# joybio/multiPrime

Measured on NVIDIA B200. Metric: candidate_x_sequence_evals_per_sec, higher is better.
Workload: dtype u32

## Files before the change

include/mpb200.h:

```cpp
#ifndef MPB200_H
#define MPB200_H

#include <stdint.h>

#ifdef __cplusplus
extern "C" {
#endif

#define MPB_ABI_VERSION 3
#define MPB_MAX_K 27
#define MPB_MAX_EXPANSIONS 65536

#define MPB_OK 0
#define MPB_EINVAL (-1)
#define MPB_ECUDA (-2)
#define MPB_ENOMEM (-3)
#define MPB_EOVERFLOW (-4)
#define MPB_EEXPAND (-5)

typedef struct mpb_ctx mpb_ctx;
typedef struct mpb_msa mpb_msa;
typedef struct mpb_hist mpb_hist;

int mpb_abi_version(void);
const char* mpb_last_error(void);
int mpb_device_count(void);

int mpb_ctx_create(int device, mpb_ctx** out);
void mpb_ctx_destroy(mpb_ctx* ctx);
int mpb_ctx_set_stream(mpb_ctx* ctx, void* cuda_stream);
int mpb_ctx_sync(mpb_ctx* ctx);
int64_t mpb_ctx_launches(mpb_ctx* ctx);
int mpb_dev_alloc(mpb_ctx* ctx, int64_t bytes, void** out);
void mpb_dev_free(mpb_ctx* ctx, void* p);
int mpb_ctx_memcpy(mpb_ctx* ctx, void* dst, const void* src, int64_t bytes);

int mpb_ctx_profile(mpb_ctx* ctx, int enable);
int mpb_ctx_profile_read(mpb_ctx* ctx, const char* kernel, double* ms, int64_t* launches, double* units);

int mpb_msa_upload(mpb_ctx* ctx, const uint8_t* packed4_hd, int64_t n_seq, int64_t n_col, int64_t row_bytes,
                   const int32_t* lens, mpb_msa** out);
void mpb_msa_free(mpb_msa* msa);
int64_t mpb_msa_nseq(const mpb_msa* msa);

int mpb_msa_set_row0(mpb_msa* msa, int64_t row0);

int mpb_seq_attr(mpb_msa* msa, int32_t* lead_gaps_hd, int32_t* rstrip_len_hd);

int mpb_window_prefilter(mpb_msa* msa, int k, int v, const int32_t* win_pos, int32_t nw, double* s0_hd, double* s1_hd);

int mpb_seq_attr_hist(mpb_msa* msa, int64_t* lead_hist_hd, int64_t* rstrip_hist_hd);

int mpb_hist_build(mpb_msa* msa, int k, int v, const int32_t* win_pos, int32_t nw, int log2_cap, mpb_hist** out);
void mpb_hist_free(mpb_hist* h);

int mpb_hist_create_empty(mpb_msa* msa, int k, int v, const int32_t* win_pos, int32_t nw, int log2_cap, mpb_hist** out);
int mpb_hist_add_counts(mpb_hist* h, const int64_t* gap_n, const int64_t* n_iupac_gap);

int mpb_hist_counts(mpb_hist* h, int64_t* gap_n, int64_t* n_iupac_gap, int64_t* n_entries);

int mpb_hist_export(mpb_hist* h, const uint8_t* sel, const int64_t* win_off, uint64_t* keys_hd, uint32_t* cnt_hd,
                    uint64_t* first_hd);

int mpb_hist_export_at(mpb_hist* h, int32_t n_sel, const int32_t* sel_idx, const int64_t* start, const int64_t* room,
                       int64_t total, uint64_t* keys_hd, uint32_t* cnt_hd, uint64_t* first_hd);

int mpb_hist_merge(mpb_hist* h, const int64_t* win_off, const uint64_t* keys_hd, const uint32_t* cnt_hd,
                   const uint64_t* first_hd);

int mpb_hist_summary(mpb_hist* h, int64_t* gap_n, double* ent, int64_t* nuniq, uint64_t* mm_key, int64_t* mm_cnt,
                     uint64_t* mm_first, int64_t* n_iupac_gap, int64_t* freq, int64_t* nn);

int mpb_hist_merge_segments(mpb_hist* h, int32_t n_seg, const int64_t* seg_off, const uint64_t* keys_hd,
                            const uint32_t* cnt_hd, const uint64_t* first_hd);

int mpb_hist_stats(mpb_hist* h, int64_t* gap_n, double* ent, int64_t* nuniq, uint64_t* mm_key, int64_t* mm_cnt,
                   uint64_t* mm_first, int64_t* n_iupac_gap);

int mpb_hist_tensors(mpb_hist* h, const uint8_t* sel, int64_t* freq_hd, int64_t* nn_hd);

int mpb_hist_dump(mpb_hist* h, int32_t w, int64_t max_n, uint64_t* keys_hd, uint32_t* cnt_hd, uint64_t* first_hd,
                  int64_t* n_out);
// ... 92 lines not shown
```

multiprime_b200/_lib.py:

```python
from __future__ import annotations

import ctypes as C
import os

import numpy as np

_PKG = os.path.dirname(os.path.abspath(__file__))
LIB_PATH = os.path.join(_PKG, "libmpb200.so")

MAX_K = 27
KEY_EMPTY = 0xFFFFFFFFFFFFFFFF
KEY_IUPAC = 0xFFFFFFFFFFFFFFFE
KEY_BASE5 = 1 << 54

_lib = None

_P = C.c_void_p
SIGNATURES = {
    "mpb_abi_version": (C.c_int, []),
    "mpb_last_error": (C.c_char_p, []),
    "mpb_device_count": (C.c_int, []),
    "mpb_ctx_create": (C.c_int, [C.c_int, C.POINTER(_P)]),
    "mpb_ctx_destroy": (None, [_P]),
    "mpb_ctx_set_stream": (C.c_int, [_P, _P]),
    "mpb_ctx_sync": (C.c_int, [_P]),
    "mpb_ctx_launches": (C.c_int64, [_P]),
    "mpb_ctx_memcpy": (C.c_int, [_P, _P, _P, C.c_int64]),
    "mpb_dev_alloc": (C.c_int, [_P, C.c_int64, C.POINTER(_P)]),
    "mpb_dev_free": (None, [_P, _P]),
    "mpb_ctx_profile": (C.c_int, [_P, C.c_int]),
    "mpb_ctx_profile_read": (C.c_int, [_P, C.c_char_p, C.POINTER(C.c_double), C.POINTER(C.c_int64),
                                        C.POINTER(C.c_double)]),
    "mpb_msa_upload": (C.c_int, [_P, _P, C.c_int64, C.c_int64, C.c_int64, _P, C.POINTER(_P)]),
    "mpb_msa_free": (None, [_P]),
    "mpb_msa_nseq": (C.c_int64, [_P]),
    "mpb_msa_set_row0": (C.c_int, [_P, C.c_int64]),
    "mpb_hist_counts": (C.c_int, [_P, _P, _P, _P]),
    "mpb_hist_export": (C.c_int, [_P, _P, _P, _P, _P, _P]),
    "mpb_seq_attr": (C.c_int, [_P, _P, _P]),
    "mpb_seq_attr_hist": (C.c_int, [_P, _P, _P]),
    "mpb_window_prefilter": (C.c_int, [_P, C.c_int, C.c_int, _P, C.c_int32, _P, _P]),
    "mpb_hist_build": (C.c_int, [_P, C.c_int, C.c_int, _P, C.c_int32, C.c_int, C.POINTER(_P)]),
    "mpb_hist_free": (None, [_P]),
    "mpb_hist_merge": (C.c_int, [_P, _P, _P, _P, _P]),
    "mpb_hist_stats": (C.c_int, [_P, _P, _P, _P, _P, _P, _P, _P]),
    "mpb_hist_tensors": (C.c_int, [_P, _P, _P, _P]),
    "mpb_hist_dump": (C.c_int, [_P, C.c_int32, C.c_int64, _P, _P, _P, C.POINTER(C.c_int64)]),
    "mpb_hist_match": (C.c_int, [_P, _P, _P, C.c_int32, _P]),
    "mpb_hist_exceptions": (C.c_int, [_P, C.c_int64, _P, _P, C.POINTER(C.c_int64)]),
    "mpb_scan": (C.c_int, [_P, C.c_int, C.c_int, C.c_uint32, C.c_uint32, _P, _P, C.c_int64, _P, _P, _P]),
    "mpb_pattern_hits": (C.c_int, [_P, C.c_int32, _P, _P, C.c_int64, _P, _P, _P, C.POINTER(C.c_int64)]),
    "mpb_seqkeys": (C.c_int, [_P, C.c_int, _P, C.c_int32, _P]),
    "mpb_tm": (C.c_int, [_P, _P, C.c_int, C.c_int64, _P, _P, _P, _P]),
    "mpb_tm_sets": (C.c_int, [_P, _P, C.c_int, C.c_int32, _P, _P, _P]),
    "mpb_walk": (C.c_int, [C.c_int, C.c_int, C.c_int, C.c_int, C.c_int32, _P, _P, _P, _P, _P, _P,
                           _P, _P, _P, _P, _P, C.c_int64, _P, _P, _P]),
    "mpb_hist_export_at": (C.c_int, [_P, C.c_int32, _P, _P, _P, C.c_int64, _P, _P, _P]),
    "mpb_hist_merge_segments": (C.c_int, [_P, C.c_int32, _P, _P, _P, _P]),
    "mpb_hist_create_empty": (C.c_int, [_P, C.c_int, C.c_int, _P, C.c_int32, C.c_int, C.POINTER(_P)]),
    "mpb_hist_add_counts": (C.c_int, [_P, _P, _P]),
    "mpb_hist_summary": (C.c_int, [_P, _P, _P, _P, _P, _P, _P, _P, _P, _P]),
    "mpb_cscan": (C.c_int, [_P, C.c_uint32, C.c_uint32, _P, C.c_int64, _P, _P, _P]),
    "mpb_walk_dev_begin": (C.c_int, [_P, C.c_int, C.c_int, C.c_uint32, C.c_uint32, C.c_int32, _P, _P, _P, _P, _P,
                                      C.POINTER(_P)]),
    "mpb_walk_dev_advance": (C.c_int, [_P]),
    "mpb_walk_dev_scan": (C.c_int, [_P]),
    "mpb_walk_dev_round": (C.c_int, [_P]),
    "mpb_walk_dev_counts": (C.c_int, [_P, C.POINTER(_P), C.POINTER(C.c_int64)]),
    "mpb_walk_dev_live": (C.c_int64, [_P]),
    "mpb_walk_dev_max_rounds": (C.c_int, [_P]),
    "mpb_walk_dev_wait": (C.c_int, [_P, C.c_int, C.POINTER(C.c_int64)]),
    "mpb_walk_dev_run": (C.c_int, [_P, C.c_int, C.POINTER(C.c_int64)]),
    "mpb_walk_dev_finish": (C.c_int, [_P, _P, _P, _P, _P, _P, C.c_int64, _P, _P, _P]),
    "mpb_walk_dev_free": (None, [_P]),
# ... 261 lines not shown
class Msa:

    def __init__(self, ctx: Context, packed4, n_seq: int, n_col: int, row_bytes: int | None = None, lens=None):
        self.ctx = ctx
        self.n_seq, self.n_col = int(n_seq), int(n_col)
        row_bytes = row_bytes if row_bytes is not None else (n_col + 1) // 2
        if lens is not None:
            lens = np.ascontiguousarray(lens, dtype=np.int32)
        h = C.c_void_p()
        check(load().mpb_msa_upload(ctx.h, ptr(packed4), n_seq, n_col, row_bytes, ptr(lens), C.byref(h)))
        self.h = h

    def close(self):
        if self.h:
            load().mpb_msa_free(self.h)
            self.h = None

    def set_row0(self, row0: int):
        check(load().mpb_msa_set_row0(self.h, row0))

    def seq_attr(self):
        lead = np.empty(self.n_seq, np.int32)
        rstrip = np.empty(self.n_seq, np.int32)
        check(load().mpb_seq_attr(self.h, ptr(lead), ptr(rstrip)))
        return lead, rstrip

    def prefilter(self, k: int, v: int, win_pos):
        win_pos = np.ascontiguousarray(win_pos, dtype=np.int32)
        s0 = np.zeros(len(win_pos), np.float64)
        s1 = np.zeros(len(win_pos), np.float64)
        check(load().mpb_window_prefilter(self.h, k, v, ptr(win_pos), len(win_pos), ptr(s0), ptr(s1)))
        return s0, s1

    def seq_attr_hist(self):
        lead = np.zeros(self.n_col + 1, np.int64)
        rstrip = np.zeros(self.n_col + 1, np.int64)
        check(load().mpb_seq_attr_hist(self.h, ptr(lead), ptr(rstrip)))
        return lead, rstrip

    def hist(self, k: int, v: int, win_pos, log2_cap: int = 0, empty: bool = False) -> "Hist":
        return Hist(self, k, v, win_pos, log2_cap, empty)

    def scan(self, k: int, v: int, fmask: int, rmask: int, cand_pos, cand_allow, bits_slot=None, counts_out=None,
             bits_out=None):
        cand_pos = np.ascontiguousarray(cand_pos, dtype=np.int32)
        cand_allow = np.ascontiguousarray(cand_allow, dtype=np.uint32).reshape(-1, 4)
        nc = len(cand_pos)
        counts = counts_out if counts_out is not None else np.zeros((nc, 3), np.int64)
        bits = bits_out
        if bits_slot is not None:
            bits_slot = np.ascontiguousarray(bits_slot, dtype=np.int32)
            nslots = int(bits_slot.max()) + 1 if nc else 0
            words = (self.n_seq + 31) // 32
            if bits is None:
                bits = np.zeros((max(nslots, 0), 3, words), np.uint32)
        if nc:
            check(load().mpb_scan(self.h, k, v, fmask, rmask, ptr(cand_pos), ptr(cand_allow), nc, ptr(counts),
                                  ptr(bits_slot), ptr(bits)))
        return counts, bits

    def pattern_hits(self, allow, lens, max_hits: int = 1 << 20):
        allow = np.ascontiguousarray(allow, dtype=np.uint32).reshape(-1, 4)
        lens = np.ascontiguousarray(lens, dtype=np.int32)
        while True:
            hp, hr, hx = (np.empty(max_hits, np.int32) for _ in range(3))
            n = C.c_int64()
            check(load().mpb_pattern_hits(self.h, len(lens), ptr(allow), ptr(lens), max_hits, ptr(hp), ptr(hr), ptr(hx),
                                          C.byref(n)))
            if n.value <= max_hits:
                break
            max_hits = int(n.value) + 16
        n = n.value
        order = np.lexsort((hx[:n], hr[:n], hp[:n]))
        return hp[:n][order], hr[:n][order], hx[:n][order]

    def seqkeys(self, k: int, win_pos) -> np.ndarray:
        win_pos = np.ascontiguousarray(win_pos, dtype=np.int32)
        out = np.empty((len(win_pos), self.n_seq), np.uint64)
        check(load().mpb_seqkeys(self.h, k, ptr(win_pos), len(win_pos), ptr(out)))
        return out


class Hist:

    def __init__(self, msa: Msa, k: int, v: int, win_pos, log2_cap: int = 0, empty: bool = False):
        self.msa = msa
        self.k, self.v = k, v
        self.win_pos = np.ascontiguousarray(win_pos, dtype=np.int32)
        self.nw = len(self.win_pos)
        self.h = None
        cap = log2_cap
        if empty:
            h = C.c_void_p()
            check(load().mpb_hist_create_empty(msa.h, k, v, ptr(self.win_pos), self.nw, cap, C.byref(h)))
            self.h = h
            self.log2_cap = cap
            return
        while True:
            h = C.c_void_p()
            rc = load().mpb_hist_build(msa.h, k, v, ptr(self.win_pos), self.nw, cap, C.byref(h))
            if rc == -4:
                if cap == 0:
                    cap = max(6, int(np.ceil(np.log2(2 * msa.n_seq + 64))))
                cap += 1
                continue
            check(rc)
            self.h = h
            self.log2_cap = cap
            break

    def close(self):
        if self.h:
            load().mpb_hist_free(self.h)
            self.h = None

    def __enter__(self):
        return self

    def __exit__(self, *a):
        self.close()

    def summary(self):
        nw, k = self.nw, self.k
        out = dict(gap_n=np.empty(nw, np.int64), ent=np.empty((nw, 4), np.float64), nuniq=np.empty((nw, 3), np.int64),
                   mm_key=np.empty(nw, np.uint64), mm_cnt=np.empty(nw, np.int64), mm_first=np.empty(nw, np.uint64),
                   n_iupac_gap=np.empty(nw, np.int64), freq=np.empty((nw, 4, k), np.int64),
                   nn=np.empty((nw, k - 1, 4, 4), np.int64))
        check(load().mpb_hist_summary(self.h, ptr(out["gap_n"]), ptr(out["ent"]), ptr(out["nuniq"]), ptr(out["mm_key"]),
                                      ptr(out["mm_cnt"]), ptr(out["mm_first"]), ptr(out["n_iupac_gap"]),
                                      ptr(out["freq"]), ptr(out["nn"])))
        return out

    def add_counts(self, gap_n, n_iupac_gap):
        gap_n = np.ascontiguousarray(gap_n, dtype=np.int64)
        n_iupac_gap = np.ascontiguousarray(n_iupac_gap, dtype=np.int64)
        check(load().mpb_hist_add_counts(self.h, ptr(gap_n), ptr(n_iupac_gap)))

# ... 347 lines not shown
```

multiprime_b200/core.py:

```python
from __future__ import annotations

import json
import math
import os
import sys
import time
from statistics import mean

import numpy as np

from . import _lib
from .comm import NoComm
from .iupac import BASES, CODE_CHARS, CHAR_CODE, allow_masks, expand_array, expand_keys, expand_strings, primer_string, rc_sets

TSV_HEADER = ["Position", "Entropy of cover (bit)", "Entropy of total (bit)", "Optimal_primer",
              "primer_degenerate_number", "nonsense_primer_number", "Optimal_coverage", "Mis-F-coverage",
              "Mis-R-coverage", "Tm", "Information"]


def _byte_table() -> bytes:
    t = bytearray(256)
    for ch, code in CHAR_CODE.items():
        if ch in "ACGTRYMKSWHBVD":
            t[ord(ch)] = code
# ... 315 lines not shown
        if row is None:
            if self._codes is not None:
                row = self._codes[s, :self.lens[s]].tobytes()
            else:
                pk = self._packed4[s]
                cells = np.empty(pk.shape[0] * 2, np.uint8)
                cells[0::2] = pk & 15
                cells[1::2] = pk >> 4
                row = cells[:self.lens[s]].tobytes()
            if len(self._row_cache) < 200000:
                self._row_cache[s] = row
        gap = b"\x00"
        w = row[p:p + k]
        if w != gap * k:
            if w.startswith(gap):
                body = w.lstrip(gap)
                g = len(w) - len(body)
                left = row[0:p].replace(gap, b"")
                if len(left) >= g:
                    w = left[len(left) - g:] + body
            if w.endswith(gap):
                body = w.rstrip(gap)
                g = len(w) - len(body)
                right = row[p + k:].replace(gap, b"")
                if len(right) >= g:
                    w = body + right[0:g]
        if len(w) < k:
            g = k - len(w)
            left = row[0:p].replace(gap, b"")
            if len(left) >= g:
                w = left[len(left) - g:] + w
        return w

    def _table_log2cap(self, k: int, n: int) -> int:
        if k < 8 or n < (1 << 17) or self.entropy_threshold > 4.0:
            return 0
        return max(10, int(math.ceil(math.log2(n / 2))))

    def design(self, positions):
        positions = [int(p) for p in positions]
        self.bit_vectors = []
        if not positions:
            return []
        per_batch = min(65535, self.windows_per_batch or _default_batch(self.n_local))
        out = []
        for b0 in range(0, len(positions), per_batch):
            out.extend(self._design_batch(positions[b0:b0 + per_batch]))
        return out

    def _design_batch(self, positions):
        k, v, N = self.primer_length, self.variation, self.total_sequence_number
        comm = self.comm
        self.stats["windows"] += len(positions)
        ph = self.stats.setdefault("phase_ms", {})
        tick = [time.perf_counter()]

        def lap(name):
            now = time.perf_counter()
            ph[name] = ph.get(name, 0.0) + 1000 * (now - tick[0])
            tick[0] = now

        if k >= 8:
            if self.n_local > 0:
                s0, s1 = self.msa.prefilter(k, v, positions)
                bound = (s0 * math.log2(self.n_local) - s1) / N
            else:
                bound = np.zeros(len(positions))
            if comm.world > 1:
                bound = comm.allreduce_sum(bound)
            keep_pos = bound <= self.entropy_threshold + 0.006
        else:
            keep_pos = np.ones(len(positions), bool)
        self.stats["prefiltered"] = self.stats.get("prefiltered", 0) + int((~keep_pos).sum())
        positions = [p for p, kp in zip(positions, keep_pos.tolist()) if kp]
        lap("prefilter")
        if not positions:
            return []
        owner = (np.arange(len(positions)) % comm.world).astype(np.int32)
        with self.msa.hist(k, v, positions, self._table_log2cap(k, self.n_local)) as hist:
            lap("hist_build")
            own = None
            try:
                if comm.world > 1:
                    st, own, mine = self._exchange(hist, positions, owner)
                    lap("exchange")
                else:
                    st, mine = hist.stats(), None
                    lap("summary")
                out = self._gates_walk_finish(hist, own, mine, owner, st, positions, lap)
            finally:
                if own is not None:
                    own.close()
        lap("free")
        return out

    def _gates_walk_finish(self, hist, own, mine, owner, st, positions, lap):
        k, v, N = self.primer_length, self.variation, self.total_sequence_number
        comm = self.comm
        gap_n = st["gap_n"]
        ratio = gap_n / N
        gap_fail = np.round(ratio, 2) >= (1 - self.coverage)
        for wi in np.nonzero(np.abs((ratio * 100) % 1 - 0.5) < 1e-6)[0]:
            gap_fail[wi] = round(int(gap_n[wi]) / N, 2) >= (1 - self.coverage)
        alive = ~gap_fail & (st["nuniq"][:, 0] >= 1)
        accepted = []
        for wi, ent in self._entropies(hist, own, mine, owner, st, positions, alive):
            accepted.append((wi, positions[wi], ent[0], ent[1], N - int(gap_n[wi]), bool(st["nuniq"][wi, 2] > 0)))
        lap("gates")
        if not accepted:
            return []
        if "freq" in st:
            freq, nn = st["freq"], st["nn"]
# ... 465 lines not shown
```

multiprime_b200/csrc/mpb200.cu:

```cuda
#include <cuda_runtime.h>
#include <stdint.h>
#include <stdarg.h>
#include <stdio.h>
#include <string.h>

#include <string>
#include <algorithm>
#include <vector>

#include "mpb200.h"
#include "mpb_host.h"
#include "mpb_device.cuh"
#include "mpb_prefilter.h"

static thread_local std::string g_err;

int mpb_fail(int code, const char* fmt, ...) {
    char buf[512];
    va_list ap;
    va_start(ap, fmt);
    vsnprintf(buf, sizeof buf, fmt, ap);
    va_end(ap);
    g_err = buf;
    return code;
// ... 793 lines not shown
                        }
                        qn += __popc(mm);
                        __syncwarp();
                    }
                }
                if (late)
                    hist_row(pl, nsp, s, len, p, k, v, kmask, row0, wi, K, C, F, E, log2cap, gap_n, iupac_gap_n, exc, exc_n,
                             exc_max, n_entries, gap_bits, nwords, spec_win, spec_row, spec_n, spec_cap, late_special ? 1 : 0, err);
            }
        }
        if (lane < gr.y) {
            const int wi = gr.x + lane;
            if (my_count)
                mpb_table_add(keys + (uint64_t)wi * cap, cnt + (uint64_t)wi * cap, first + (uint64_t)wi * cap, log2cap, my_major,
                              my_count, my_first, err, &n_entries[wi], elist + (uint64_t)wi * cap);
            if (my_gaps) atomicAdd(&gap_n[wi], (unsigned long long)my_gaps);
        }
    }
    hist_flush(s_qkey[warp], s_qmeta[warp], qn, lane, keys, cnt, first, elist, n_entries, log2cap, row0, row_base, err);
    __syncthreads();
    const unsigned nd = s_ndefer < HIST_DEFER_CAP ? s_ndefer : HIST_DEFER_CAP;
    for (unsigned i = threadIdx.x; i < nd; i += HIST_THREADS) {
        const unsigned e = s_defer[i];
        const unsigned ws = e >> 13;
        const int wi = groups[blockIdx.y + (int)(ws >> 5) * gridDim.y].x + (int)(ws & 31u);
        const int64_t s = row_base + (e & 0xFFFu);
        hist_row(pl, nsp, s, lens[s], win_pos[wi], k, v, kmask, row0, wi, keys + (uint64_t)wi * cap, cnt + (uint64_t)wi * cap,
                 first + (uint64_t)wi * cap, elist + (uint64_t)wi * cap, log2cap, gap_n, iupac_gap_n, exc, exc_n, exc_max,
                 n_entries, gap_bits, nwords, spec_win, spec_row, spec_n, spec_cap, (e & 0x1000u) != 0u ? 1 : 0, err);
    }
}

__global__ void __launch_bounds__(256)
k_prefilter_sums(const unsigned int* __restrict__ bins, double* __restrict__ s0, double* __restrict__ s1) {
    const unsigned int* B = bins + (long long)blockIdx.x * PRE_BINS;
    double a0 = 0, a1 = 0;
    for (int i = threadIdx.x; i < PRE_BINS; i += 256) {
        const unsigned int c = B[i];
        if (c) {
            a0 += (double)c;
            if (c > 1) a1 += (double)c * log2((double)c);
        }
    }
    __shared__ double sh0[8], sh1[8];
    for (int o = 16; o > 0; o >>= 1) {
        a0 += __shfl_xor_sync(0xffffffffu, a0, o);
        a1 += __shfl_xor_sync(0xffffffffu, a1, o);
    }
    if ((threadIdx.x & 31) == 0) {
        sh0[threadIdx.x >> 5] = a0;
        sh1[threadIdx.x >> 5] = a1;
    }
    __syncthreads();
    if (threadIdx.x == 0) {
        for (int w = 1; w < 8; ++w) {
            a0 += sh0[w];
            a1 += sh1[w];
        }
        s0[blockIdx.x] = a0;
        s1[blockIdx.x] = a1;
    }
}

#define CW_THREADS 256
#define CW_WARPS (CW_THREADS / 32)
#define CW_WPW 16
#define CW_WORDS (CW_WARPS * CW_WPW)
#define CW_ROWS (CW_WORDS * 32)
#define CW_QCAP 10240
#define CW_QROOM 7680

struct ColClass {
    uint32_t plain, agp, match;
};

__device__ __forceinline__ ColClass col_classify(uint32_t A, uint32_t C, uint32_t G, uint32_t T, int cb, int k, int L,
// ... 277 lines not shown
        }
        chunks.push_back(c);
    }
}

static bool mpb_use_col_passes() {
    const char* e = getenv("MPB_WINPASS");
    return !(e && strcmp(e, "row") == 0);
}

template <class Kern>
static unsigned window_pass_gy(mpb_ctx* ctx, Kern kern, unsigned gx, int nw) {
    int per_sm = 1;
    if (cudaOccupancyMaxActiveBlocksPerMultiprocessor(&per_sm, kern, HIST_THREADS, 0) != cudaSuccess || per_sm < 1) per_sm = 1;
    const long long resident = (long long)per_sm * ctx->sm_count;
    if ((long long)gx * nw <= 16 * resident) return (unsigned)nw;
    long long lo = (resident + gx - 1) / gx, hi = (4 * resident + gx - 1) / gx + 1;
    if (lo < 1) lo = 1;
    if (hi > nw) hi = nw;
    if (lo > hi) lo = hi;
    unsigned best = (unsigned)lo;
    double best_eff = -1;
    for (long long gy = lo; gy <= hi; ++gy) {
        const long long blocks = (long long)gx * gy, waves = (blocks + resident - 1) / resident;
        const double eff = (double)blocks / (double)(waves * resident);
        if (eff >= best_eff) {
            best_eff = eff;
            best = (unsigned)gy;
        }
    }
    return best;
}

extern "C" int mpb_window_prefilter(mpb_msa* m, int k, int v, const int32_t* win_pos, int32_t nw, double* s0_hd,
                                    double* s1_hd) {
    if (!m || !win_pos || !s0_hd || !s1_hd) return fail(MPB_EINVAL, "NULL argument");
    if (k < 8 || k > MPB_MAX_K || v < 0 || nw < 1) return fail(MPB_EINVAL, "prefilter needs 8 <= k <= %d", MPB_MAX_K);
    for (int i = 0; i < nw; ++i)
        if (win_pos[i] < 0 || win_pos[i] >= m->n_col)
            return fail(MPB_EINVAL, "win_pos[%d]=%d outside the alignment", i, win_pos[i]);
    mpb_ctx* ctx = m->ctx;
    CK(cudaSetDevice(ctx->device));
    bool inside = true;
    for (int i = 0; i < nw; ++i) inside = inside && win_pos[i] + k <= m->n_col;
    if (mpb_use_col_passes() && inside && !m->short_rows) return mpb_prefilter_bs(m, k, v, win_pos, nw, s0_hd, s1_hd);
    unsigned int* bins = nullptr;
    CK(cudaMallocAsync(&bins, (size_t)nw * PRE_BINS * 4, ctx->stream));
    CK(cudaMemsetAsync(bins, 0, (size_t)nw * PRE_BINS * 4, ctx->stream));
    InBuf wp(ctx, win_pos, (size_t)nw * 4);
    OutBuf o0(ctx, s0_hd, (size_t)nw * 8), o1(ctx, s1_hd, (size_t)nw * 8);
    if (wp.rc || o0.rc || o1.rc) return MPB_ECUDA;
    {
        const unsigned gx = (unsigned)((m->n_seq + (long long)WIN_ROWS - 1) / (long long)WIN_ROWS);
        std::vector<int2> groups;
        mpb_window_groups(win_pos, nw, groups);
        InBuf gr(ctx, groups.data(), groups.size() * sizeof(int2));
        if (gr.rc) return gr.rc;
        const unsigned gy = window_pass_gy(ctx, k_prefilter, gx, (int)groups.size());
        ctx->pending_units = (double)nw * (double)m->n_seq;
        LAUNCH(ctx, k_prefilter, dim3(gx, gy), HIST_THREADS, 0, m->planes, m->nsp, m->n_seq, m->lens, k, v, wp.dev<int32_t>(),
               gr.dev<int2>(), (int)groups.size(), bins, m->err);
    }
    LAUNCH(ctx, k_prefilter_sums, (unsigned)nw, 256, 0, bins, o0.dev<double>(), o1.dev<double>());
    CK(o0.finish());
    CK(o1.finish());
    CK(cudaFreeAsync(bins, ctx->stream));
    return mpb_check_flags(ctx, m->err);
}

static int hist_alloc_spec(mpb_hist* h, int64_t spec_cap) {
    mpb_ctx* ctx = h->msa->ctx;
    h->spec_cap = spec_cap;
    cudaError_t e = cudaMallocAsync(&h->spec_win, (size_t)h->nw * spec_cap * sizeof(uint4), ctx->stream);
    if (e == cudaSuccess) e = cudaMallocAsync(&h->spec_row, (size_t)h->nw * spec_cap * 4, ctx->stream);
    if (e != cudaSuccess) return fail(MPB_ENOMEM, "special-row lists (%d windows x %lld rows): %s", h->nw, (long long)spec_cap,
                                      cudaGetErrorString(e));
    return 0;
}

static int hist_launch_build(mpb_hist* h) {
    mpb_msa* m = h->msa;
    mpb_ctx* ctx = m->ctx;
    const int nw = h->nw;
    const uint64_t slots = (uint64_t)nw << h->log2cap;
    CK(cudaMemsetAsync(h->keys, 0xFF, slots * 8, ctx->stream));
    CK(cudaMemsetAsync(h->cnt, 0, slots * 4, ctx->stream));
    CK(cudaMemsetAsync(h->first, 0xFF, slots * 8, ctx->stream));
    CK(cudaMemsetAsync(h->gap_n, 0, (size_t)nw * 8, ctx->stream));
    CK(cudaMemsetAsync(h->iupac_gap_n, 0, (size_t)nw * 8, ctx->stream));
    CK(cudaMemsetAsync(h->n_entries, 0, (size_t)nw * 8, ctx->stream));
    CK(cudaMemsetAsync(h->spec_n, 0, (size_t)nw * 8, ctx->stream));
    CK(cudaMemsetAsync(h->exc_n, 0, 8, ctx->stream));
    if (mpb_use_col_passes()) {
        std::vector<int2> chunks;
        std::vector<int32_t> chunk_win;
        mpb_window_chunks(h->h_win_pos.data(), nw, h->k, chunks, chunk_win);
        InBuf cd(ctx, chunks.data(), chunks.size() * sizeof(int2)), cw(ctx, chunk_win.data(), chunk_win.size() * 4);
        if (cd.rc || cw.rc) return MPB_ECUDA;
        HistOut o;
        o.keys = h->keys;
// ... 72 lines not shown
    if (e == cudaSuccess) e = cudaMallocAsync(&h->exc_n, 8, ctx->stream);
    if (e == cudaSuccess) e = cudaMallocAsync(&h->spec_bits, (size_t)nw * m->nwords * 4, ctx->stream);
    if (e == cudaSuccess) e = cudaMallocAsync(&h->gap_bits, (size_t)nw * m->nwords * 4, ctx->stream);
    if (e == cudaSuccess) e = cudaMallocAsync(&h->freq, (size_t)nw * 4 * k * 8, ctx->stream);
    if (e == cudaSuccess) e = cudaMallocAsync(&h->nn, (size_t)nw * (k - 1) * 16 * 8, ctx->stream);
    if (e != cudaSuccess) {
        mpb_hist_free(h);
        return fail(MPB_ENOMEM, "haplotype tables (%d windows x 2^%d slots): %s", nw, log2_cap, cudaGetErrorString(e));
    }
    CK(cudaMemcpyAsync(h->win_pos, h->h_win_pos.data(), (size_t)nw * 4, cudaMemcpyHostToDevice, ctx->stream));
    if (!fill) {
        const uint64_t sl = (uint64_t)nw << log2_cap;
        CK(cudaMemsetAsync(h->keys, 0xFF, sl * 8, ctx->stream));
        CK(cudaMemsetAsync(h->cnt, 0, sl * 4, ctx->stream));
        CK(cudaMemsetAsync(h->first, 0xFF, sl * 8, ctx->stream));
        CK(cudaMemsetAsync(h->gap_n, 0, (size_t)nw * 8, ctx->stream));
        CK(cudaMemsetAsync(h->iupac_gap_n, 0, (size_t)nw * 8, ctx->stream));
        CK(cudaMemsetAsync(h->n_entries, 0, (size_t)nw * 8, ctx->stream));
        CK(cudaMemsetAsync(h->spec_n, 0, (size_t)nw * 8, ctx->stream));
        CK(cudaMemsetAsync(h->exc_n, 0, 8, ctx->stream));
        *out = h;
        return 0;
    }
    int64_t cap = m->n_seq / 32;
    if (cap < 1024) cap = m->n_seq < 1024 ? m->n_seq : 1024;
    for (int attempt = 0; attempt < 2; ++attempt) {
        int rc = hist_alloc_spec(h, cap);
        if (rc == 0) rc = hist_launch_build(h);
        if (rc == 0) rc = mpb_check_flags(ctx, m->err);
        if (rc) {
            mpb_hist_free(h);
            return rc;
        }
        std::vector<unsigned long long> sn(nw);
        CK(cudaMemcpyAsync(sn.data(), h->spec_n, (size_t)nw * 8, cudaMemcpyDeviceToHost, ctx->stream));
        CK(cudaStreamSynchronize(ctx->stream));
        unsigned long long mx = 0;
        for (auto x : sn) mx = x > mx ? x : mx;
        if ((int64_t)mx <= cap) break;
        if (attempt == 1) {
            mpb_hist_free(h);
            return fail(MPB_EOVERFLOW, "special-row list overflow after resize");
        }
        cudaFreeAsync(h->spec_win, ctx->stream);
        cudaFreeAsync(h->spec_row, ctx->stream);
        h->spec_win = nullptr;
        h->spec_row = nullptr;
        cap = (int64_t)mx;
    }
    *out = h;
    return 0;
}

extern "C" int mpb_hist_build(mpb_msa* m, int k, int v, const int32_t* win_pos, int32_t nw, int log2_cap,
                              mpb_hist** out) {
    return hist_create(m, k, v, win_pos, nw, log2_cap, 1, out);
}

extern "C" int mpb_hist_create_empty(mpb_msa* m, int k, int v, const int32_t* win_pos, int32_t nw, int log2_cap,
                                     mpb_hist** out) {
    return hist_create(m, k, v, win_pos, nw, log2_cap, 0, out);
}

extern "C" int mpb_hist_counts(mpb_hist* h, int64_t* gap_n, int64_t* n_iupac_gap, int64_t* n_entries) {
    if (!h) return fail(MPB_EINVAL, "NULL argument");
    mpb_ctx* ctx = h->msa->ctx;
    CK(cudaSetDevice(ctx->device));
    const size_t bytes = (size_t)h->nw * 8;
    if (gap_n) CK(cudaMemcpyAsync(gap_n, h->gap_n, bytes, cudaMemcpyDeviceToHost, ctx->stream));
    if (n_iupac_gap) CK(cudaMemcpyAsync(n_iupac_gap, h->iupac_gap_n, bytes, cudaMemcpyDeviceToHost, ctx->stream));
    if (n_entries) CK(cudaMemcpyAsync(n_entries, h->n_entries, bytes, cudaMemcpyDeviceToHost, ctx->stream));
// ... 1006 lines not shown
```

multiprime_b200/csrc/mpb_host.h:

```cpp
#pragma once
#include <cuda_runtime.h>
#include <stdarg.h>
#include <stdint.h>
#include <stdio.h>
#include <string.h>

#include <map>
#include <string>
#include <vector>

#include "mpb200.h"

int mpb_fail(int code, const char* fmt, ...);

#define MPB_CK(call)                                                                                   \
    do {                                                                                               \
        cudaError_t e__ = (call);                                                                      \
        if (e__ != cudaSuccess)                                                                        \
            return mpb_fail(e__ == cudaErrorMemoryAllocation ? MPB_ENOMEM : MPB_ECUDA, "%s:%d %s: %s", \
                            __FILE__, __LINE__, #call, cudaGetErrorString(e__));                       \
    } while (0)

struct ProfRec {
    const char* name;
    cudaEvent_t e0, e1;
    double units;
};
#define MPB_CTX_PINNED_INTS 256
struct mpb_ctx {
    int device;
    cudaStream_t stream;
    cudaStream_t copy_stream;
    int* pinned;
    int64_t launches;
    int sm_count;
    bool profile;
    std::vector<ProfRec> recs;
    std::map<std::string, double> extra_units;
    double pending_units;
};
static inline int mpb_ctx_device(mpb_ctx* c) { return c->device; }
static inline cudaStream_t mpb_ctx_stream(mpb_ctx* c) { return c->stream; }
static inline int mpb_ctx_sms(mpb_ctx* c) { return c->sm_count; }

#define MPB_LAUNCH_NAMED(ctx, name, kern, grid, block, smem, ...)                 \
    do {                                                                          \
// ... 128 lines not shown
```

multiprime_b200/csrc/mpb_prefilter.cu:

```cuda
#include <cooperative_groups.h>
#include <cuda_runtime.h>
#include <stdint.h>
#include <string.h>

#include <vector>

#include "mpb200.h"
#include "mpb_host.h"
#include "mpb_device.cuh"
#include "mpb_prefilter.h"

namespace cg = cooperative_groups;

#define fail mpb_fail
#define CK MPB_CK

#define BS_BITS 13
#define BS_BINS (1 << BS_BITS)
#define BS_THREADS 256
#define BS_CLUSTER 8
#define BS_DEFER 2048

constexpr uint16_t BS_LO[27] = {0x414, 0x1900, 0x32, 0x13, 0xc40, 0xc4, 0x602, 0x1088, 0x4a0, 0xd, 0x1401, 0x409, 0x1a0, 0x248,
                                0x1204, 0x184, 0x100c, 0x1028, 0x1104, 0x1018, 0x58, 0x1006, 0x118, 0x881, 0xc8, 0x482, 0x504};
// ... 53 lines not shown
    if (!mpb_load_window(pl, nsp, s, len, p, k, kmask, w)) atomicOr(err, MPB_ERR_SHORT_ROW);
    const bool isgap = __popc(w.gapv) > v;
    if (w.multi == 0 || isgap) {
        uint32_t c = w.c, g = w.g, tt = w.t;
        if (w.multi) {
            const uint32_t a = w.a;
            c &= ~a;
            g &= ~(a | c);
            tt &= ~(a | c | g);
        }
        atomicAdd(&s_bins[bs_code(c, g, tt)], 1u);
    } else {
        const uint32_t total = mpb_expansions(w);
        if (total > MPB_MAX_EXP) {
            atomicOr(err, MPB_ERR_EXPAND);
        } else {
            for (uint32_t e = 0; e < total; ++e) {
                uint32_t a, c, g, tt;
                mpb_expand(w, e, a, c, g, tt);
                atomicAdd(&s_bins[bs_code(c, g, tt)], 1u);
            }
        }
    }
}

__global__ void __cluster_dims__(BS_CLUSTER, 1, 1) __launch_bounds__(BS_THREADS, 4)
k_prefilter_bs(const uint32_t* __restrict__ colp, long long nwords, const uint8_t* __restrict__ cons,
               const uint32_t* __restrict__ pl, int64_t nsp, int64_t n_seq, const int32_t* __restrict__ lens, int k, int v,
               const int32_t* __restrict__ win_pos, double* __restrict__ part, int* __restrict__ err) {
    __shared__ unsigned int s_bins[BS_BINS];
    __shared__ unsigned int s_def[BS_DEFER];
    __shared__ unsigned int s_ndef;
    __shared__ unsigned int s_major;
    __shared__ double s_red[2][BS_THREADS / 32];
    cg::cluster_group cluster = cg::this_cluster();
    const unsigned rank = cluster.block_rank();
    const int wi = blockIdx.x / BS_CLUSTER;
    const int p = win_pos[wi];
    const uint32_t kmask = (1u << k) - 1u;
    for (int i = threadIdx.x; i < BS_BINS; i += BS_THREADS) s_bins[i] = 0;
    if (threadIdx.x == 0) {
        s_ndef = 0;
        uint32_t lo = 0, hi = 0;
        for (int j = 0; j < k; ++j) {
            const uint32_t b = cons[p + j];
            lo |= (b & 1u) << j;
            hi |= ((b >> 1) & 1u) << j;
        }
        s_major = bs_code(lo & ~hi, hi & ~lo, lo & hi);
    }
    __syncthreads();
    const uint32_t major = s_major;
    const long long n_w = (n_seq + 31) / 32;
    const long long per = (n_w + BS_CLUSTER - 1) / BS_CLUSTER;
    const long long w_lo = (long long)rank * per, w_hi = (w_lo + per < n_w) ? w_lo + per : n_w;
    const uint32_t* __restrict__ col0 = colp + ((long long)p * 4) * nwords;
    unsigned my_count = 0;
    for (long long W = w_lo + threadIdx.x; W < w_hi; W += BS_THREADS) {
        const long long left = (long long)n_seq - W * 32;
        const uint32_t vm = left >= 32 ? 0xFFFFFFFFu : ((1u << left) - 1u);
        uint32_t H[16];
#pragma unroll
        for (int i = 0; i < 16; ++i) H[i] = 0;
        BsAcc a = {0u, 0xFFFFFFFFu, 0u, 0u, 0u};
        bs_cols<0>(col0, nwords, (unsigned)W, k, H, a);
        const uint32_t special = ((a.gfirst | a.glast) & ~a.allgap) | a.anymul;
        const uint32_t plain = ~special & vm;
// ... 10 lines not shown
            BS_SWAP(0, 2, 0x33333333u) BS_SWAP(1, 2, 0x33333333u) BS_SWAP(4, 2, 0x33333333u) BS_SWAP(5, 2, 0x33333333u)
            BS_SWAP(8, 2, 0x33333333u) BS_SWAP(9, 2, 0x33333333u) BS_SWAP(12, 2, 0x33333333u) BS_SWAP(13, 2, 0x33333333u)
            BS_SWAP(0, 1, 0x55555555u) BS_SWAP(2, 1, 0x55555555u) BS_SWAP(4, 1, 0x55555555u) BS_SWAP(6, 1, 0x55555555u)
            BS_SWAP(8, 1, 0x55555555u) BS_SWAP(10, 1, 0x55555555u) BS_SWAP(12, 1, 0x55555555u) BS_SWAP(14, 1, 0x55555555u)
#pragma unroll
            for (int r = 0; r < 16; ++r) {
                if ((rest >> r) & 1u) atomicAdd(&s_bins[H[r] & 0xFFFFu], 1u);
                if ((rest >> (r + 16)) & 1u) atomicAdd(&s_bins[H[r] >> 16], 1u);
            }
        }
        uint32_t sp = special & vm;
        while (sp) {
            const int r = __ffs(sp) - 1;
            sp &= sp - 1;
            const int64_t s = W * 32 + r;
            const unsigned idx = atomicAdd(&s_ndef, 1u);
            if (idx < BS_DEFER) s_def[idx] = (unsigned)s;
            else bs_slow_row(pl, nsp, s, lens[s], p, k, kmask, v, s_bins, err);
        }
    }
    my_count = __reduce_add_sync(0xffffffffu, my_count);
    if ((threadIdx.x & 31) == 0 && my_count) atomicAdd(&s_bins[major], my_count);
    __syncthreads();
    const unsigned nd = s_ndef < BS_DEFER ? s_ndef : BS_DEFER;
    for (unsigned i = threadIdx.x; i < nd; i += BS_THREADS) {
        const int64_t s = (int64_t)s_def[i];
        bs_slow_row(pl, nsp, s, lens[s], p, k, kmask, v, s_bins, err);
    }
    cluster.sync();
    const unsigned int* rb[BS_CLUSTER];
#pragma unroll
    for (int q = 0; q < BS_CLUSTER; ++q) rb[q] = cluster.map_shared_rank(s_bins, q);
    double a0 = 0, a1 = 0;
    const int slice = BS_BINS / BS_CLUSTER;
    for (int i = (int)rank * slice + threadIdx.x; i < ((int)rank + 1) * slice; i += BS_THREADS) {
        unsigned c = 0;
#pragma unroll
        for (int q = 0; q < BS_CLUSTER; ++q) c += rb[q][i];
        if (c) {
            a0 += (double)c;
            if (c > 1) a1 += (double)c * log2((double)c);
        }
    }
    for (int o = 16; o > 0; o >>= 1) {
        a0 += __shfl_xor_sync(0xffffffffu, a0, o);
        a1 += __shfl_xor_sync(0xffffffffu, a1, o);
    }
    if ((threadIdx.x & 31) == 0) {
        s_red[0][threadIdx.x >> 5] = a0;
        s_red[1][threadIdx.x >> 5] = a1;
    }
    __syncthreads();
    if (threadIdx.x == 0) {
        for (int w = 1; w < BS_THREADS / 32; ++w) {
            a0 += s_red[0][w];
            a1 += s_red[1][w];
        }
        part[((long long)wi * BS_CLUSTER + rank) * 2] = a0;
        part[((long long)wi * BS_CLUSTER + rank) * 2 + 1] = a1;
    }
    cluster.sync();
}

int mpb_prefilter_bs(mpb_msa* m, int k, int v, const int32_t* win_pos, int32_t nw, double* s0_hd, double* s1_hd) {
    mpb_ctx* ctx = m->ctx;
    InBuf wp(ctx, win_pos, (size_t)nw * 4);
    if (wp.rc) return wp.rc;
    double* part = nullptr;
    CK(cudaMallocAsync(&part, (size_t)nw * BS_CLUSTER * 2 * sizeof(double), ctx->stream));
    ctx->pending_units = (double)nw * (double)m->n_seq;
    MPB_LAUNCH_NAMED(ctx, "k_prefilter", k_prefilter_bs, (unsigned)nw * BS_CLUSTER, BS_THREADS, 0, m->colp, (long long)m->nwords,
                     m->cons, m->planes, m->nsp, m->n_seq, m->lens, k, v, wp.dev<int32_t>(), part, m->err);
    std::vector<double> hp((size_t)nw * BS_CLUSTER * 2);
    CK(cudaMemcpyAsync(hp.data(), part, hp.size() * sizeof(double), cudaMemcpyDeviceToHost, ctx->stream));
    CK(cudaFreeAsync(part, ctx->stream));
    int rc = mpb_check_flags(ctx, m->err);
    if (rc) return rc;
    const bool dev_out = mpb_is_device_ptr(s0_hd);
    std::vector<double> s0(nw), s1(nw);
    for (int w = 0; w < nw; ++w) {
        double a0 = 0, a1 = 0;
        for (int r = 0; r < BS_CLUSTER; ++r) {
            a0 += hp[((size_t)w * BS_CLUSTER + r) * 2];
            a1 += hp[((size_t)w * BS_CLUSTER + r) * 2 + 1];
        }
        s0[w] = a0;
        s1[w] = a1;
    }
    if (dev_out) {
        CK(cudaMemcpyAsync(s0_hd, s0.data(), (size_t)nw * 8, cudaMemcpyHostToDevice, ctx->stream));
        CK(cudaMemcpyAsync(s1_hd, s1.data(), (size_t)nw * 8, cudaMemcpyHostToDevice, ctx->stream));
        CK(cudaStreamSynchronize(ctx->stream));
    } else {
        memcpy(s0_hd, s0.data(), (size_t)nw * 8);
        memcpy(s1_hd, s1.data(), (size_t)nw * 8);
    }
    return 0;
}
```

multiprime_b200/csrc/mpb_prefilter.h:

```cpp
#pragma once
#include <stdint.h>

#include "mpb200.h"
#include "mpb_host.h"

int mpb_prefilter_bs(mpb_msa* m, int k, int v, const int32_t* win_pos, int32_t nw, double* s0_hd, double* s1_hd);
```

Baseline: 160.6 billion.

## Size haplotype hash table from prefilter linear-count distinct estimate

The prefilter kernels now also count occupied bins per window, and a linear-counting estimate of distinct k-mers per window is returned to Python. The hash table log2 capacity is then chosen from the largest kept window's estimate, with a floor of 2^12 and the old heuristic as a ceiling, replacing the fixed heuristic. This shrinks the table so build, scan and clear touch less memory. In exchange an underestimate can trigger rebuilds, and a new three-quarters-full check forces an overflow retry.

Measured after the change: 165.0 billion (median of 6 runs). 1.03x the previous value.

```diff
diff --git a/include/mpb200.h b/include/mpb200.h
--- a/include/mpb200.h
+++ b/include/mpb200.h
@@ -48,6 +48,8 @@
 int mpb_seq_attr(mpb_msa* msa, int32_t* lead_gaps_hd, int32_t* rstrip_len_hd);
 
 int mpb_window_prefilter(mpb_msa* msa, int k, int v, const int32_t* win_pos, int32_t nw, double* s0_hd, double* s1_hd);
+int mpb_window_prefilter_distinct(mpb_msa* msa, int k, int v, const int32_t* win_pos, int32_t nw, double* s0_hd,
+                                  double* s1_hd, double* distinct_h);
 
 int mpb_seq_attr_hist(mpb_msa* msa, int64_t* lead_hist_hd, int64_t* rstrip_hist_hd);
 
diff --git a/multiprime_b200/_lib.py b/multiprime_b200/_lib.py
--- a/multiprime_b200/_lib.py
+++ b/multiprime_b200/_lib.py
@@ -40,6 +40,7 @@
     "mpb_seq_attr": (C.c_int, [_P, _P, _P]),
     "mpb_seq_attr_hist": (C.c_int, [_P, _P, _P]),
     "mpb_window_prefilter": (C.c_int, [_P, C.c_int, C.c_int, _P, C.c_int32, _P, _P]),
+    "mpb_window_prefilter_distinct": (C.c_int, [_P, C.c_int, C.c_int, _P, C.c_int32, _P, _P, _P]),
     "mpb_hist_build": (C.c_int, [_P, C.c_int, C.c_int, _P, C.c_int32, C.c_int, C.POINTER(_P)]),
     "mpb_hist_free": (None, [_P]),
     "mpb_hist_merge": (C.c_int, [_P, _P, _P, _P, _P]),
@@ -367,6 +368,13 @@
         check(load().mpb_window_prefilter(self.h, k, v, ptr(win_pos), len(win_pos), ptr(s0), ptr(s1)))
         return s0, s1
 
+    def prefilter_distinct(self, k: int, v: int, win_pos):
+        win_pos = np.ascontiguousarray(win_pos, dtype=np.int32)
+        s0, s1, distinct = (np.zeros(len(win_pos), np.float64) for _ in range(3))
+        check(load().mpb_window_prefilter_distinct(self.h, k, v, ptr(win_pos), len(win_pos), ptr(s0), ptr(s1),
+                                                   ptr(distinct)))
+        return s0, s1, distinct
+
     def seq_attr_hist(self):
         lead = np.zeros(self.n_col + 1, np.int64)
         rstrip = np.zeros(self.n_col + 1, np.int64)
@@ -424,6 +432,7 @@
         self.win_pos = np.ascontiguousarray(win_pos, dtype=np.int32)
         self.nw = len(self.win_pos)
         self.h = None
+        self.rebuilds = 0
         cap = log2_cap
         if empty:
             h = C.c_void_p()
@@ -438,6 +447,7 @@
                 if cap == 0:
                     cap = max(6, int(np.ceil(np.log2(2 * msa.n_seq + 64))))
                 cap += 1
+                self.rebuilds += 1
                 continue
             check(rc)
             self.h = h
diff --git a/multiprime_b200/core.py b/multiprime_b200/core.py
--- a/multiprime_b200/core.py
+++ b/multiprime_b200/core.py
@@ -371,10 +371,18 @@
                 w = left[len(left) - g:] + w
         return w
 
-    def _table_log2cap(self, k: int, n: int) -> int:
+    TABLE_MIN_LOG2 = 12
+
+    def _table_log2cap(self, k: int, n: int, distinct=None) -> int:
         if k < 8 or n < (1 << 17) or self.entropy_threshold > 4.0:
-            return 0
-        return max(10, int(math.ceil(math.log2(n / 2))))
+            ceiling = 0
+        else:
+            ceiling = max(10, int(math.ceil(math.log2(n / 2))))
+        if distinct is None or not len(distinct) or not np.isfinite(distinct).all():
+            return ceiling
+        ceiling = ceiling or max(6, int(math.ceil(math.log2(2 * n + 64))))
+        need = max(self.TABLE_MIN_LOG2, int(math.ceil(math.log2(2 * float(distinct.max()) + 64))))
+        return min(need, ceiling)
 
     def design(self, positions):
         positions = [int(p) for p in positions]
@@ -399,9 +407,13 @@
             ph[name] = ph.get(name, 0.0) + 1000 * (now - tick[0])
             tick[0] = now
 
+        distinct = None
         if k >= 8:
             if self.n_local > 0:
-                s0, s1 = self.msa.prefilter(k, v, positions)
+                if hasattr(self.msa, "prefilter_distinct"):
+                    s0, s1, distinct = self.msa.prefilter_distinct(k, v, positions)
+                else:
+                    s0, s1 = self.msa.prefilter(k, v, positions)
                 bound = (s0 * math.log2(self.n_local) - s1) / N
             else:
                 bound = np.zeros(len(positions))
@@ -416,7 +428,9 @@
         if not positions:
             return []
         owner = (np.arange(len(positions)) % comm.world).astype(np.int32)
-        with self.msa.hist(k, v, positions, self._table_log2cap(k, self.n_local)) as hist:
+        log2cap = self._table_log2cap(k, self.n_local, None if distinct is None else distinct[keep_pos])
+        with self.msa.hist(k, v, positions, log2cap) as hist:
+            self.stats["table_rebuilds"] = self.stats.get("table_rebuilds", 0) + getattr(hist, "rebuilds", 0)
             lap("hist_build")
             own = None
             try:
diff --git a/multiprime_b200/csrc/mpb200.cu b/multiprime_b200/csrc/mpb200.cu
--- a/multiprime_b200/csrc/mpb200.cu
+++ b/multiprime_b200/csrc/mpb200.cu
@@ -849,16 +849,21 @@
 }
 
 __global__ void __launch_bounds__(256)
-k_prefilter_sums(const unsigned int* __restrict__ bins, double* __restrict__ s0, double* __restrict__ s1) {
+k_prefilter_sums(const unsigned int* __restrict__ bins, double* __restrict__ s0, double* __restrict__ s1,
+                 unsigned int* __restrict__ occupied) {
     const unsigned int* B = bins + (long long)blockIdx.x * PRE_BINS;
     double a0 = 0, a1 = 0;
+    unsigned occ = 0;
     for (int i = threadIdx.x; i < PRE_BINS; i += 256) {
         const unsigned int c = B[i];
         if (c) {
             a0 += (double)c;
             if (c > 1) a1 += (double)c * log2((double)c);
-        }
-    }
+            ++occ;
+        }
+    }
+    occ = __reduce_add_sync(0xffffffffu, occ);
+    if ((threadIdx.x & 31) == 0 && occ) atomicAdd(&occupied[blockIdx.x], occ);
     __shared__ double sh0[8], sh1[8];
     for (int o = 16; o > 0; o >>= 1) {
         a0 += __shfl_xor_sync(0xffffffffu, a0, o);
@@ -1202,8 +1207,8 @@
     return best;
 }
 
-extern "C" int mpb_window_prefilter(mpb_msa* m, int k, int v, const int32_t* win_pos, int32_t nw, double* s0_hd,
-                                    double* s1_hd) {
+extern "C" int mpb_window_prefilter_distinct(mpb_msa* m, int k, int v, const int32_t* win_pos, int32_t nw, double* s0_hd,
+                                             double* s1_hd, double* distinct_h) {
     if (!m || !win_pos || !s0_hd || !s1_hd) return fail(MPB_EINVAL, "NULL argument");
     if (k < 8 || k > MPB_MAX_K || v < 0 || nw < 1) return fail(MPB_EINVAL, "prefilter needs 8 <= k <= %d", MPB_MAX_K);
     for (int i = 0; i < nw; ++i)
@@ -1213,10 +1218,14 @@
     CK(cudaSetDevice(ctx->device));
     bool inside = true;
     for (int i = 0; i < nw; ++i) inside = inside && win_pos[i] + k <= m->n_col;
-    if (mpb_use_col_passes() && inside && !m->short_rows) return mpb_prefilter_bs(m, k, v, win_pos, nw, s0_hd, s1_hd);
+    if (mpb_use_col_passes() && inside && !m->short_rows)
+        return mpb_prefilter_bs(m, k, v, win_pos, nw, s0_hd, s1_hd, distinct_h);
     unsigned int* bins = nullptr;
+    unsigned int* occupied = nullptr;
     CK(cudaMallocAsync(&bins, (size_t)nw * PRE_BINS * 4, ctx->stream));
     CK(cudaMemsetAsync(bins, 0, (size_t)nw * PRE_BINS * 4, ctx->stream));
+    CK(cudaMallocAsync(&occupied, (size_t)nw * 4, ctx->stream));
+    CK(cudaMemsetAsync(occupied, 0, (size_t)nw * 4, ctx->stream));
     InBuf wp(ctx, win_pos, (size_t)nw * 4);
     OutBuf o0(ctx, s0_hd, (size_t)nw * 8), o1(ctx, s1_hd, (size_t)nw * 8);
     if (wp.rc || o0.rc || o1.rc) return MPB_ECUDA;
@@ -1231,11 +1240,22 @@
         LAUNCH(ctx, k_prefilter, dim3(gx, gy), HIST_THREADS, 0, m->planes, m->nsp, m->n_seq, m->lens, k, v, wp.dev<int32_t>(),
                gr.dev<int2>(), (int)groups.size(), bins, m->err);
     }
-    LAUNCH(ctx, k_prefilter_sums, (unsigned)nw, 256, 0, bins, o0.dev<double>(), o1.dev<double>());
+    LAUNCH(ctx, k_prefilter_sums, (unsigned)nw, 256, 0, bins, o0.dev<double>(), o1.dev<double>(), occupied);
     CK(o0.finish());
     CK(o1.finish());
+    std::vector<unsigned int> occ(nw);
+    CK(cudaMemcpyAsync(occ.data(), occupied, (size_t)nw * 4, cudaMemcpyDeviceToHost, ctx->stream));
     CK(cudaFreeAsync(bins, ctx->stream));
-    return mpb_check_flags(ctx, m->err);
+    CK(cudaFreeAsync(occupied, ctx->stream));
+    const int rc = mpb_check_flags(ctx, m->err);
+    if (rc == 0 && distinct_h)
+        for (int w = 0; w < nw; ++w) distinct_h[w] = mpb_linear_count(occ[w], PRE_BINS);
+    return rc;
+}
+
+extern "C" int mpb_window_prefilter(mpb_msa* m, int k, int v, const int32_t* win_pos, int32_t nw, double* s0_hd,
+                                    double* s1_hd) {
+    return mpb_window_prefilter_distinct(m, k, v, win_pos, nw, s0_hd, s1_hd, nullptr);
 }
 
 static int hist_alloc_spec(mpb_hist* h, int64_t spec_cap) {
@@ -1374,11 +1394,17 @@
             mpb_hist_free(h);
             return rc;
         }
-        std::vector<unsigned long long> sn(nw);
+        std::vector<unsigned long long> sn(nw), ne(nw);
         CK(cudaMemcpyAsync(sn.data(), h->spec_n, (size_t)nw * 8, cudaMemcpyDeviceToHost, ctx->stream));
+        CK(cudaMemcpyAsync(ne.data(), h->n_entries, (size_t)nw * 8, cudaMemcpyDeviceToHost, ctx->stream));
         CK(cudaStreamSynchronize(ctx->stream));
-        unsigned long long mx = 0;
+        unsigned long long mx = 0, most = 0;
         for (auto x : sn) mx = x > mx ? x : mx;
+        for (auto x : ne) most = x > most ? x : most;
+        if (most > (3ull << log2_cap) / 4) {
+            mpb_hist_free(h);
+            return fail(MPB_EOVERFLOW, "haplotype table past 3/4 full (%llu entries, 2^%d slots)", most, log2_cap);
+        }
         if ((int64_t)mx <= cap) break;
         if (attempt == 1) {
             mpb_hist_free(h);
diff --git a/multiprime_b200/csrc/mpb_host.h b/multiprime_b200/csrc/mpb_host.h
--- a/multiprime_b200/csrc/mpb_host.h
+++ b/multiprime_b200/csrc/mpb_host.h
@@ -1,5 +1,6 @@
 #pragma once
 #include <cuda_runtime.h>
+#include <math.h>
 #include <stdarg.h>
 #include <stdint.h>
 #include <stdio.h>
@@ -12,6 +13,10 @@
 #include "mpb200.h"
 
 int mpb_fail(int code, const char* fmt, ...);
+
+static inline double mpb_linear_count(double occupied, double bins) {
+    return occupied >= bins ? HUGE_VAL : -bins * log1p(-occupied / bins);
+}
 
 #define MPB_CK(call)                                                                                   \
     do {                                                                                               \
diff --git a/multiprime_b200/csrc/mpb_prefilter.cu b/multiprime_b200/csrc/mpb_prefilter.cu
--- a/multiprime_b200/csrc/mpb_prefilter.cu
+++ b/multiprime_b200/csrc/mpb_prefilter.cu
@@ -109,7 +109,7 @@
     __shared__ unsigned int s_def[BS_DEFER];
     __shared__ unsigned int s_ndef;
     __shared__ unsigned int s_major;
-    __shared__ double s_red[2][BS_THREADS / 32];
+    __shared__ double s_red[3][BS_THREADS / 32];
     cg::cluster_group cluster = cg::this_cluster();
     const unsigned rank = cluster.block_rank();
     const int wi = blockIdx.x / BS_CLUSTER;
@@ -186,6 +186,7 @@
 #pragma unroll
     for (int q = 0; q < BS_CLUSTER; ++q) rb[q] = cluster.map_shared_rank(s_bins, q);
     double a0 = 0, a1 = 0;
+    unsigned occ = 0;
     const int slice = BS_BINS / BS_CLUSTER;
     for (int i = (int)rank * slice + threadIdx.x; i < ((int)rank + 1) * slice; i += BS_THREADS) {
         unsigned c = 0;
@@ -194,38 +195,46 @@
         if (c) {
             a0 += (double)c;
             if (c > 1) a1 += (double)c * log2((double)c);
+            ++occ;
         }
     }
     for (int o = 16; o > 0; o >>= 1) {
         a0 += __shfl_xor_sync(0xffffffffu, a0, o);
         a1 += __shfl_xor_sync(0xffffffffu, a1, o);
     }
+    occ = __reduce_add_sync(0xffffffffu, occ);
     if ((threadIdx.x & 31) == 0) {
         s_red[0][threadIdx.x >> 5] = a0;
         s_red[1][threadIdx.x >> 5] = a1;
+        s_red[2][threadIdx.x >> 5] = (double)occ;
     }
     __syncthreads();
     if (threadIdx.x == 0) {
+        double a2 = occ;
         for (int w = 1; w < BS_THREADS / 32; ++w) {
             a0 += s_red[0][w];
             a1 += s_red[1][w];
-        }
-        part[((long long)wi * BS_CLUSTER + rank) * 2] = a0;
-        part[((long long)wi * BS_CLUSTER + rank) * 2 + 1] = a1;
+            a2 += s_red[2][w];
+        }
+        double* o = part + ((long long)wi * BS_CLUSTER + rank) * 3;
+        o[0] = a0;
+        o[1] = a1;
+        o[2] = a2;
     }
     cluster.sync();
 }
 
-int mpb_prefilter_bs(mpb_msa* m, int k, int v, const int32_t* win_pos, int32_t nw, double* s0_hd, double* s1_hd) {
+int mpb_prefilter_bs(mpb_msa* m, int k, int v, const int32_t* win_pos, int32_t nw, double* s0_hd, double* s1_hd,
+                     double* distinct) {
     mpb_ctx* ctx = m->ctx;
     InBuf wp(ctx, win_pos, (size_t)nw * 4);
     if (wp.rc) return wp.rc;
     double* part = nullptr;
-    CK(cudaMallocAsync(&part, (size_t)nw * BS_CLUSTER * 2 * sizeof(double), ctx->stream));
+    CK(cudaMallocAsync(&part, (size_t)nw * BS_CLUSTER * 3 * sizeof(double), ctx->stream));
     ctx->pending_units = (double)nw * (double)m->n_seq;
     MPB_LAUNCH_NAMED(ctx, "k_prefilter", k_prefilter_bs, (unsigned)nw * BS_CLUSTER, BS_THREADS, 0, m->colp, (long long)m->nwords,
                      m->cons, m->planes, m->nsp, m->n_seq, m->lens, k, v, wp.dev<int32_t>(), part, m->err);
-    std::vector<double> hp((size_t)nw * BS_CLUSTER * 2);
+    std::vector<double> hp((size_t)nw * BS_CLUSTER * 3);
     CK(cudaMemcpyAsync(hp.data(), part, hp.size() * sizeof(double), cudaMemcpyDeviceToHost, ctx->stream));
     CK(cudaFreeAsync(part, ctx->stream));
     int rc = mpb_check_flags(ctx, m->err);
@@ -233,13 +242,15 @@
     const bool dev_out = mpb_is_device_ptr(s0_hd);
     std::vector<double> s0(nw), s1(nw);
     for (int w = 0; w < nw; ++w) {
-        double a0 = 0, a1 = 0;
+        double a0 = 0, a1 = 0, occ = 0;
         for (int r = 0; r < BS_CLUSTER; ++r) {
-            a0 += hp[((size_t)w * BS_CLUSTER + r) * 2];
-            a1 += hp[((size_t)w * BS_CLUSTER + r) * 2 + 1];
+            a0 += hp[((size_t)w * BS_CLUSTER + r) * 3];
+            a1 += hp[((size_t)w * BS_CLUSTER + r) * 3 + 1];
+            occ += hp[((size_t)w * BS_CLUSTER + r) * 3 + 2];
         }
         s0[w] = a0;
         s1[w] = a1;
+        if (distinct) distinct[w] = mpb_linear_count(occ, BS_BINS);
     }
     if (dev_out) {
         CK(cudaMemcpyAsync(s0_hd, s0.data(), (size_t)nw * 8, cudaMemcpyHostToDevice, ctx->stream));
diff --git a/multiprime_b200/csrc/mpb_prefilter.h b/multiprime_b200/csrc/mpb_prefilter.h
--- a/multiprime_b200/csrc/mpb_prefilter.h
+++ b/multiprime_b200/csrc/mpb_prefilter.h
@@ -4,4 +4,5 @@
 #include "mpb200.h"
 #include "mpb_host.h"
 
-int mpb_prefilter_bs(mpb_msa* m, int k, int v, const int32_t* win_pos, int32_t nw, double* s0_hd, double* s1_hd);
+int mpb_prefilter_bs(mpb_msa* m, int k, int v, const int32_t* win_pos, int32_t nw, double* s0_hd, double* s1_hd,
+                     double* distinct);
```
